# pranoyr/attention-models

Hardware: AMD Instinct MI355X
Metric: ViTVQGAN 256px train-step images/sec (higher is better)
Workload: dtype f32; 1 GPU; BASELINE.json configs[2]: ViTVQGAN dim=256 patch=8 img=256 depth=6+6 h=8 d=64 mlp=2048 (SwiGLU), codebook 8192x32; GAN train step (D phase + G phase, gradient penalty, per_loss_weight=0), Adam, clip 1.0; global_batch=32, batch_per_gpu=32, parallelism=dp1

## Files before the change

attention-models_amd/amk/dense.py:

```python
import ctypes

import torch

from . import lib as _lib
from .lib import EPI_BIAS, EPI_RESID, EPI_SWIGLU, EPI_SWIGLU_BWD, GEMM_NN, GEMM_NT, GEMM_TN, GemmDesc


def _p(t):
    return ctypes.c_void_p(t.data_ptr()) if t is not None else ctypes.c_void_p(0)


def _stream():
    return ctypes.c_void_p(torch.cuda.current_stream().cuda_stream)


def _mat(t, what):
    if t is None:
        return None
    if not t.is_cuda:
        raise RuntimeError("amk ops run only on MI355X (HIP) tensors; got a CPU tensor. There is no CPU fallback.")
    if t.dtype != torch.float32:
        raise RuntimeError(f"amk kernels compute in fp32; got {t.dtype} for {what}")
    if t.dim() != 2:
        raise RuntimeError(f"{what} must be a matrix, got shape {tuple(t.shape)}")
# ... 175 lines not shown
        rows.append([src, R, K, H, blk, dst_w, dst_wt, NR])
        spans.append((dst_w, nw, dst_wt, nt))
        blk += (_pad32(R) // 32) * (_pad32(K) // 32)
    return torch.tensor(rows, dtype=torch.int64).view(-1, 8), blk, off, spans


def x6_split_table(flat, table_dev, n_blocks, planes):
    rc = _lib.load().amk_gemm_x6_split_table(_p(flat), flat.numel(), _p(table_dev), table_dev.shape[0], n_blocks,
                                             _p(planes), planes.numel(), _stream())
    _lib.check(rc, "amk_gemm_x6_split_table")


def gemm_x6_nt(a, planes, N, bias=None, *, a2=None, planes2=None):
    a, a2 = _mat(a, "a"), _mat(a2, "a2")
    M, K = a.shape
    c = torch.empty((M, N), device=a.device, dtype=torch.float32)
    L = _lib.load()
    if a2 is not None:
        if bias is not None or a2.shape[0] != M:
            raise RuntimeError("gemm_x6_nt: the two-segment form takes no bias and equal row counts")
        rc = L.amk_gemm_x6_nt2(_p(a), a.stride(0), _p(planes), K, _p(a2), a2.stride(0), _p(planes2), a2.shape[1],
                               _p(c), N, M, N, _stream())
        _lib.check(rc, "amk_gemm_x6_nt2")
        return c
    rc = L.amk_gemm_x6_nt(_p(a), a.stride(0), _p(planes), _p(_vec(bias, N, "bias")), _p(c), N, M, N, K, _stream())
    _lib.check(rc, "amk_gemm_x6_nt")
    return c


def gemm_x6_nt_swiglu(a, gate_planes, H, b12=None, *, keep_ab=True):
    a = _mat(a, "a")
    M, K = a.shape
    gate = torch.empty((M, H), device=a.device, dtype=torch.float32)
    ab = torch.empty((M, 2 * H), device=a.device, dtype=torch.float32) if keep_ab else None
    rc = _lib.load().amk_gemm_x6_nt_swiglu(_p(a), a.stride(0), _p(gate_planes), _p(_vec(b12, 2 * H, "b12")), _p(gate), H,
                                           _p(ab), 2 * H, M, H, K, _stream())
    _lib.check(rc, "amk_gemm_x6_nt_swiglu")
    return gate, ab


def gemm_x6_nt_swiglu_bwd(dy, w3t_planes, ab):
    dy, ab = _mat(dy, "dy"), _mat(ab, "ab")
    M, K = dy.shape
    H = ab.shape[1] // 2
    if ab.shape != (M, 2 * H):
        raise RuntimeError(f"gemm_x6_nt_swiglu_bwd: (a | b) {tuple(ab.shape)} against dy {tuple(dy.shape)}")
    d_ab = torch.empty((M, 2 * H), device=dy.device, dtype=torch.float32)
    rc = _lib.load().amk_gemm_x6_nt_swiglu_bwd(_p(dy), dy.stride(0), _p(w3t_planes), _p(ab), ab.stride(0), _p(d_ab), 2 * H,
                                               M, H, K, _stream())
    _lib.check(rc, "amk_gemm_x6_nt_swiglu_bwd")
    return d_ab


def _mat16(t, what):
    if not t.is_cuda:
        raise RuntimeError("amk ops run only on MI355X (HIP) tensors; got a CPU tensor. There is no CPU fallback.")
    if t.dtype != torch.bfloat16 or t.dim() != 2:
        raise RuntimeError(f"{what} must be a bf16 matrix, got {t.dtype} {tuple(t.shape)}")
    if t.stride(1) != 1 or t.stride(0) % 8 or t.data_ptr() % 16:
        t = t.contiguous()
    return t


def supported_bf16(N, K):
    return N > 0 and K > 0 and N % 8 == 0 and K % 8 == 0


def gemm_tn_bf16(y, x, want_bias=False, out=None, bias_out=None):
    y, x = _mat16(y, "y"), _mat16(x, "x")
    M, N = y.shape
    K = x.shape[1]
    if x.shape[0] != M:
        raise RuntimeError(f"gemm_tn_bf16: y has {M} rows, x {x.shape[0]}")
    if not supported_bf16(N, K):
        raise RuntimeError(f"gemm_tn_bf16: N and K must be multiples of 8, got {N}, {K}")
    L = _lib.load()
    dw = _out(out, (N, K), "gemm_tn_bf16 out")
    if dw is None:
        dw = torch.empty(N, K, device=y.device, dtype=torch.float32)
    db = None
    if want_bias:
        db = _out(bias_out, (N,), "gemm_tn_bf16 bias_out")
        if db is None:
            db = torch.empty(N, device=y.device, dtype=torch.float32)
    nbytes = L.amk_gemm_tn_bf16_ws_bytes(M, N, K)
    ws = torch.empty(nbytes // 4, device=y.device, dtype=torch.float32) if nbytes else None
    rc = L.amk_gemm_tn_bf16(_p(y), y.stride(0), _p(x), x.stride(0), _p(dw), K, _p(db), M, N, K, _p(ws), nbytes, _stream())
    _lib.check(rc, "amk_gemm_tn_bf16")
    return dw, db


def _bias32(bias, n):
    if bias is None:
        return None
    if bias.dtype != torch.float32 or not bias.is_cuda:
        raise RuntimeError("gemm bf16: the bias stays in fp32 (it is added to the fp32 accumulators)")
    bias = bias.contiguous()
    if bias.numel() != n or bias.data_ptr() % 16:
        raise RuntimeError(f"gemm bf16: bias of {bias.numel()} elements (16-byte aligned) expected {n}")
    return bias


def gemm_nt_bf16(a, w, bias=None):
    a, w = _mat16(a, "a"), _mat16(w, "w")
    (M, K), N = a.shape, w.shape[0]
    if w.shape[1] != K or not supported_bf16(N, K):
# ... 47 lines not shown
```

attention-models_amd/amk/lib.py:

```python
import ctypes
import os
import re

_HERE = os.path.dirname(os.path.abspath(__file__))
LIB_PATH = os.environ.get("AMK_LIB") or os.path.join(_HERE, "libamk.so")
HEADER_PATH = os.path.normpath(os.path.join(_HERE, "..", "..", "include", "amk.h"))

AMK_OK = 0

_c = ctypes
_P = _c.c_void_p
_I = _c.c_int
_L = _c.c_int64
_F = _c.c_float



class GemmDesc(_c.Structure):
    _fields_ = [("op", _c.c_int32), ("epilogue", _c.c_int32), ("m", _L),
                ("n", _c.c_int32), ("k", _c.c_int32), ("split", _c.c_int32), ("reserved", _c.c_int32),
                ("a", _P), ("a2", _P), ("w", _P), ("w2", _P), ("c", _P), ("c2", _P),
                ("lda", _L), ("lda2", _L), ("ldw", _L), ("ldw2", _L), ("ldc", _L), ("ldc2", _L),
                ("bias", _P), ("bias2", _P), ("resid", _P), ("ldr", _L),
                ("ln_mean", _P), ("ln_rstd", _P), ("ln_gamma", _P), ("ln_beta", _P),
# ... 6 lines not shown
SIGNATURES = {
    "amk_version": (_I, []),
    "amk_arch": (_c.c_char_p, []),
    "amk_last_error": (_c.c_char_p, []),
    "amk_attn_fwd": (_I, [_P] * 7 + [_I] * 5 + [_L] * 12 + [_F, _P]),
    "amk_attn_scores_bytes": (_L, [_I, _I, _I, _I]),
    "amk_attn_fwd_keep": (_I, [_P] * 8 + [_I] * 5 + [_L] * 12 + [_F, _P]),
    "amk_attn_fwd_x6_ws_bytes": (_L, [_I, _I, _I]),
    "amk_attn_fwd_x6": (_I, [_P] * 8 + [_I] * 5 + [_L] * 12 + [_F, _P]),
    "amk_attn_fwd_x6_keep": (_I, [_P] * 9 + [_I] * 5 + [_L] * 12 + [_F, _P]),
    "amk_attn_decode_ws_floats": (_L, [_I, _I, _I, _I]),
    "amk_attn_decode": (_I, [_P] * 9 + [_I] * 4 + [_L] * 9 + [_F, _P]),
    "amk_attn_decode_bf16": (_I, [_P] * 9 + [_I] * 4 + [_L] * 9 + [_F, _P]),
    "amk_gemm_rows_bf16": (_I, [_P, _L, _P, _L, _P, _P, _L, _I, _I, _I, _I, _P]),
    "amk_attn_bwd_ws_floats": (_L, [_I, _I, _I, _I, _I]),
    "amk_attn_bwd": (_I, [_P] * 12 + [_I] * 5 + [_L] * 24 + [_F, _I, _P]),
    "amk_attn_bwd_kept": (_I, [_P] * 13 + [_I] * 5 + [_L] * 24 + [_F, _I, _P]),
    "amk_vq_num_partials": (_L, [_L]),
    "amk_vq_lookup_fwd": (_I, [_P, _P, _L, _I, _I, _I] + [_P] * 9 + [_P]),
    "amk_vq_lookup_bwd": (_I, [_P] * 7 + [_F, _L, _I, _I, _P, _P, _P]),
    "amk_vq_lookup_bwd_rows": (_I, [_P] * 7 + [_F, _L, _I, _I, _P, _P, _P]),
    "amk_vq_padded_codes": (_I, [_I, _I]),
    "amk_vq_gather": (_I, [_P, _P, _L, _I, _I, _P, _P, _P]),
    "amk_agent_num_chunks": (_I, [_I]),
    "amk_agent_ws_floats": (_L, [_I, _I, _I, _I, _I]),
    "amk_agent_num_chunks_dh": (_I, [_I, _I]),
    "amk_agent_ws_floats_dh": (_L, [_I, _I, _I, _I, _I, _I]),
    "amk_agent_attn_fwd": (_I, [_P] * 10 + [_I] * 5 + [_L] * 12 + [_F, _P]),
    "amk_agent_attn_bwd": (_I, [_P] * 14 + [_I] * 5 + [_L] * 21 + [_F, _P]),
    "amk_agent_conv_grad_reduce": (_I, [_P, _P, _L, _I, _P, _P, _P]),
    "amk_agent_bf16_ws_floats": (_L, [_I, _I, _I, _I, _I, _I]),
    "amk_agent_attn_bf16_fwd": (_I, [_P] * 10 + [_I] * 5 + [_L] * 12 + [_F, _P]),
    "amk_agent_attn_bf16_bwd": (_I, [_P] * 14 + [_I] * 5 + [_L] * 21 + [_F, _P]),
    "amk_rowsum_num_partials": (_I, [_L]),
    "amk_add_layernorm_fwd": (_I, [_P, _P, _P, _P, _L, _I, _F, _P, _P, _P, _P, _P]),
    "amk_add_layernorm_bwd": (_I, [_P, _P, _P, _P, _P, _P, _L, _I, _P, _P, _P]),
    "amk_colsum": (_I, [_P, _L, _I, _P, _P]),
    "amk_swiglu_fwd": (_I, [_P, _L, _I, _P, _P]),
    "amk_swiglu_bwd": (_I, [_P, _P, _L, _I, _P, _P]),
    "amk_geglu_fwd": (_I, [_P, _L, _I, _P, _P]),
    "amk_geglu_bwd": (_I, [_P, _P, _L, _I, _P, _P]),
    "amk_opt_num_partials": (_I, []),
    "amk_sumsq_partials": (_I, [_P, _L, _P, _P]),
    "amk_adam_flat_step": (_I, [_P] * 4 + [_L, _P, _P, _P, _I] + [_F] * 6 + [_I, _P, _P]),
    "amk_adam_flat_step_shadow": (_I, [_P] * 4 + [_L, _P, _P, _P, _I] + [_F] * 6 + [_I, _P, _P, _P]),
    "amk_gemm_x6_planes_bytes": (_L, [_I, _I]),
    "amk_gemm_x6_split": (_I, [_P, _L, _I, _I, _P, _P]),
    "amk_gemm_x6_nt": (_I, [_P, _L, _P, _P, _P, _L, _I, _I, _I, _P]),
    "amk_gemm_x6_nt2": (_I, [_P, _L, _P, _I, _P, _L, _P, _I, _P, _L, _I, _I, _P]),
    "amk_gemm_x6_gate_rows": (_I, [_I]),
    "amk_gemm_x6_nt_swiglu": (_I, [_P, _L, _P, _P, _P, _L, _P, _L, _I, _I, _I, _P]),
    "amk_gemm_x6_nt_swiglu_bwd": (_I, [_P, _L, _P, _P, _L, _P, _L, _I, _I, _I, _P]),
    "amk_gemm_x6_split_table": (_I, [_P, _L, _P, _I, _L, _P, _L, _P]),
    "amk_gemm_f32_ws_bytes": (_L, [_c.POINTER(GemmDesc)]),
    "amk_gemm_f32": (_I, [_c.POINTER(GemmDesc), _P, _L, _P]),
    "amk_row_stats": (_I, [_P, _L, _I, _F, _P, _P, _P]),
    "amk_attn_bf16_fwd": (_I, [_P] * 7 + [_I] * 5 + [_L] * 12 + [_F, _P]),
    "amk_attn_bf16_bwd_ws_floats": (_L, [_I, _I, _I, _I]),
    "amk_attn_bf16_bwd": (_I, [_P] * 12 + [_I] * 5 + [_L] * 24 + [_F, _P]),
    "amk_swiglu_bf16_fwd": (_I, [_P, _L, _I, _P, _P]),
    "amk_swiglu_bf16_bwd": (_I, [_P, _P, _L, _I, _P, _P]),
    "amk_add_layernorm_mixed_fwd": (_I, [_P, _I, _P, _P, _P, _L, _I, _F, _P, _P, _P, _P, _P]),
    "amk_add_layernorm_mixed_bwd": (_I, [_P, _I, _P, _P, _P, _P, _P, _L, _I, _P, _P, _P, _P]),
    "amk_geglu_ln_bf16_num_partials": (_I, [_L, _I]),
    "amk_geglu_ln_bf16_fwd": (_I, [_P, _L, _L, _I, _P, _P, _F, _P, _P, _P, _P]),
    "amk_geglu_ln_bf16_bwd": (_I, [_P, _L, _P, _P, _P, _P, _L, _I, _P, _P, _P]),
    "amk_gemm_bf16": (_I, [_I, _I, _P, _L, _P, _L, _P, _P, _L, _P, _L, _L, _I, _I, _P]),
    "amk_gemm_bf16_swiglu_bwd": (_I, [_P, _L, _P, _L, _P, _L, _P, _L, _L, _I, _I, _P]),
    "amk_gemm_tn_bf16_ws_bytes": (_L, [_L, _I, _I]),
    "amk_gemm_tn_bf16": (_I, [_P, _L, _P, _L, _P, _L, _P, _L, _I, _I, _P, _L, _P]),
    "amk_sample_step": (_I, [_P, _P, _F, _P, _c.c_uint64, _c.c_uint64, _F, _L, _I, _I, _P, _F, _P, _P, _P]),
    "amk_moe_route_ws_ints": (_L, [_L, _I, _I]),
    "amk_moe_route": (_I, [_P, _L, _I, _I] + [_P] * 8),
    "amk_grouped_gemm_nt": (_I, [_P, _L, _I, _P, _P, _P, _P, _L, _I, _I, _I, _P, _P]),
    "amk_grouped_gemm_nn": (_I, [_P, _L, _I, _P, _P, _P, _P, _L, _I, _I, _I, _P, _P]),
    "amk_grouped_gemm_nt_acc": (_I, [_P, _L, _I, _P, _P, _P, _P, _L, _I, _I, _I, _P, _I, _P]),
    "amk_grouped_gemm_nn_acc": (_I, [_P, _L, _I, _P, _P, _P, _P, _L, _I, _I, _I, _P, _I, _P]),
    "amk_grouped_gemm_wgrad": (_I, [_P, _L, _I, _P, _L, _I, _P, _P, _P, _L, _I, _I, _I, _P, _P, _P]),
    "amk_moe_combine": (_I, [_P, _P, _P, _L, _I, _I, _I, _P, _P]),
    "amk_moe_expert_sums": (_I, [_P, _L, _I, _P, _P, _L, _I, _I, _I, _P, _P]),
    "amk_moe_topk": (_I, [_P, _L, _I, _I, _P, _P, _P]),
    "amk_moe_route_distinct": (_I, [_P, _L, _I, _I, _P, _P, _P, _P]),
    "amk_moe_combine_rows": (_I, [_P, _P, _P, _L, _I, _I, _I, _I, _I, _P, _P]),
    "amk_moe_gate_grad_rows": (_I, [_P, _P, _P, _P, _L, _I, _I, _I, _I, _I, _P, _P]),
    "amk_moe_gate_grad": (_I, [_P, _P, _P, _P, _L, _I, _I, _I, _I, _P, _P]),
    "amk_bnact_ws_floats": (_L, [_I, _I, _L]),
    "amk_bnact_fwd": (_I, [_P, _P, _P, _I, _I, _L, _F, _F, _F] + [_P] * 7),
    "amk_bnact_bwd": (_I, [_P] * 6 + [_I, _I, _L, _F] + [_P] * 6),
    "amk_bnact_bwd_bwd": (_I, [_P] * 10 + [_I, _I, _L, _F] + [_P] * 5),
    "amk_bnact_bf16_fwd": (_I, [_P, _P, _P, _I, _I, _L, _F, _F, _F] + [_P] * 7),
    "amk_bnact_bf16_bwd": (_I, [_P] * 6 + [_I, _I, _L, _F] + [_P] * 6),
    "amk_bnact_bf16_bwd_bwd": (_I, [_P] * 10 + [_I, _I, _L, _F] + [_P] * 5),
    "amk_gnact_ws_floats": (_L, [_I, _I, _L, _I]),
    "amk_gnact_fwd": (_I, [_P, _P, _P, _I, _I, _L, _I, _F, _I] + [_P] * 5),
    "amk_gnact_bwd": (_I, [_P] * 6 + [_I, _I, _L, _I, _I] + [_P] * 5),
    "amk_gnact_bf16_ws_floats": (_L, [_I, _I, _L, _I]),
    "amk_gnact_bf16_fwd": (_I, [_P, _P, _P, _I, _I, _L, _I, _F, _I] + [_P] * 5),
    "amk_gnact_bf16_bwd": (_I, [_P] * 6 + [_I, _I, _L, _I, _I] + [_P] * 5),
    "amk_ce_head_fwd_ws_bytes": (_L, [_L, _I, _I]),
    "amk_ce_head_bwd_ws_bytes": (_L, [_L, _I, _I]),
    "amk_ce_head_fwd": (_I, [_P, _L, _P, _L, _P, _L, _L, _I, _I, _P, _P, _P, _P, _P, _L, _P]),
    "amk_ce_head_bwd": (_I, [_P, _L, _P, _L, _P, _L, _L, _I, _I, _P, _P, _P, _P, _P, _L, _P, _L, _P, _L, _P]),
    "amk_ce_head_bias_fwd": (_I, [_P, _L, _P, _L, _P, _P, _L, _L, _I, _I, _P, _P, _P, _P, _P, _L, _P]),
    "amk_ce_head_bias_bwd": (_I, [_P, _L, _P, _L, _P, _P, _L, _L, _I, _I, _P, _P, _P, _P, _P, _L, _P, _L, _P, _P, _L, _P]),
    "amk_ce_head_bf16_fwd_ws_bytes": (_L, [_L, _I, _I]),
    "amk_ce_head_bf16_bwd_ws_bytes": (_L, [_L, _I, _I]),
# ... 48 lines not shown
```

attention-models_amd/amk/ops.py:

```python
import ctypes
import os
import weakref

import torch
from torch.autograd.function import once_differentiable

from . import lib as _lib

_NULL = ctypes.c_void_p(0)


def _ptr(t):
    return ctypes.c_void_p(t.data_ptr()) if t is not None else _NULL


def _stream():
    return ctypes.c_void_p(torch.cuda.current_stream().cuda_stream)


KERNEL_EVENTS = None


class _timed:

# ... 1507 lines not shown
    if not _ln_supported(x.shape[-1]) or x.numel() == 0 or not x.is_cuda:
        return torch.nn.functional.layer_norm(x, (x.shape[-1],), weight, bias, eps)
    if branch and _mixed_ln():
        with torch.autocast("cuda", enabled=False):
            return _AddLayerNormMixed.apply(x, None, weight, bias, eps)[1]
    return _LayerNorm.apply(x, weight, bias, eps)


def add_layer_norm(x, res, weight, bias, eps=1e-5, branch=False):
    if not _ln_supported(x.shape[-1]) or x.numel() == 0 or not x.is_cuda:
        h = x + res
        return h, torch.nn.functional.layer_norm(h, (h.shape[-1],), weight, bias, eps)
    if branch and _mixed_ln():
        with torch.autocast("cuda", enabled=False):
            return _AddLayerNormMixed.apply(x, res.float(), weight, bias, eps)
    return _AddLayerNorm.apply(x, res, weight, bias, eps)


def colsum(x2):
    M, N = x2.shape
    if N % 4 != 0 or N > 1024:
        return x2.sum(0)
    x2 = _c16(x2)
    L = _lib.load()
    part = torch.empty((L.amk_rowsum_num_partials(M), N), device=x2.device, dtype=torch.float32)
    _lib.check(L.amk_colsum(_ptr(x2), M, N, _ptr(part), _stream()), "amk_colsum")
    return part.sum(0)


class _BiasLinear(torch.autograd.Function):

    @staticmethod
    def forward(ctx, x, weight, bias):
        _require_device(x, weight, bias)
        ctx.save_for_backward(x, weight)
        return torch.nn.functional.linear(x, weight, bias)

    @staticmethod
    @once_differentiable
    def backward(ctx, dy):
        x, weight = ctx.saved_tensors
        dy2 = dy.contiguous().view(-1, dy.shape[-1])
        dx = dy2.mm(weight).view(x.shape) if ctx.needs_input_grad[0] else None
        dw = dy2.t().mm(x.reshape(-1, x.shape[-1])) if ctx.needs_input_grad[1] else None
        db = colsum(dy2) if ctx.needs_input_grad[2] else None
        return dx, dw, db


GEMM_MODE = os.environ.get("AMK_GEMM", "auto")
if GEMM_MODE not in ("auto", "f32", "bf16x6"):
    raise RuntimeError(f"AMK_GEMM must be auto, f32 or bf16x6 (got {GEMM_MODE!r})")
X6_LINEAR = os.environ.get("AMK_X6_LINEAR", "1") != "0"
X6_AUTO_KINDS = frozenset(k for k in os.environ.get("AMK_X6_KINDS", "linear,linear2,ffn").split(",") if k)
X6_AUTO_FORMS = frozenset(k for k in os.environ.get("AMK_X6_FORMS", "fwd").split(",") if k)


def gemm_x6_nt(a2, b2, bias=None):
    _require_device(a2, b2, bias)
    if a2.stride(1) != 1:
        a2 = a2.contiguous()
    if b2.stride(1) != 1:
        b2 = b2.contiguous()
    M, K = a2.shape
    N = b2.shape[0]
    L = _lib.load()
    planes = torch.empty((L.amk_gemm_x6_planes_bytes(N, K),), device=a2.device, dtype=torch.uint8)
    c = torch.empty((M, N), device=a2.device, dtype=torch.float32)
    with _timed(f"gemm_x6_nt M{M} N{N} K{K}"):
        _lib.check(L.amk_gemm_x6_split(_ptr(b2), b2.stride(0), N, K, _ptr(planes), _stream()), "amk_gemm_x6_split")
        rc = L.amk_gemm_x6_nt(_ptr(a2), a2.stride(0), _ptr(planes), _ptr(bias), _ptr(c), N, M, N, K, _stream())
    _lib.check(rc, "amk_gemm_x6_nt")
    return c


def _x6_ok(x, weight):
    K = weight.shape[1]
    if K % 4 or x.numel() == 0 or x.data_ptr() % 16 or weight.data_ptr() % 16:
        return False
    if x.stride(-1) != 1 or (x.dim() >= 2 and x.stride(-2) % 4):
        return False
    return x.numel() * 4 < 0x7ffffff0 and weight.numel() * 8 < 0x7ffffff0


class _LinearX6(torch.autograd.Function):

    @staticmethod
    def forward(ctx, x, weight, bias):
        _require_device(x, weight, bias)
        x2 = x.reshape(-1, x.shape[-1])
        ctx.save_for_backward(x2, weight)
        ctx.x_shape = x.shape
        ctx.has_bias = bias is not None
        return gemm_x6_nt(x2, weight, bias).view(*x.shape[:-1], weight.shape[0])

    @staticmethod
    @once_differentiable
    def backward(ctx, dy):
        x2, weight = ctx.saved_tensors
        dy2 = dy.contiguous().view(-1, dy.shape[-1])
        dx = dw = db = None
        if ctx.needs_input_grad[0]:
            N = weight.shape[0]
            if N % 4 == 0:
                dx = gemm_x6_nt(dy2, weight.t().contiguous()).view(ctx.x_shape)
            else:
                dx = dy2.mm(weight).view(ctx.x_shape)
        if ctx.needs_input_grad[1]:
            dw = dy2.t().mm(x2)
        if ctx.has_bias and ctx.needs_input_grad[2]:
            db = colsum(dy2)
        return dx, dw, db


def _x6_planes(kind, x, *weights, gate=None):
    if GEMM_MODE != "auto" or not X6_LINEAR or kind not in X6_AUTO_KINDS or torch.is_autocast_enabled():
        return None
    if not x.is_cuda or x.dtype != torch.float32 or x.numel() == 0 or x.shape[-1] % 4:
        return None
    if kind == "linear" and min(weights[0].shape) < 128:
        return None
    out = []
    for w in weights:
        pl = getattr(w, "_amk_x6", None)
        if pl is None or w._version != w._amk_x6_version or pl.gate != (w is gate) or (pl.R, pl.K) != tuple(w.shape):
            return None
        out.append(pl)
    return tuple(out)


class _X6Linear(torch.autograd.Function):

    @staticmethod
    def forward(ctx, x, weight, bias, pl):
        from . import dense

        x2 = x.reshape(-1, x.shape[-1])
        ctx.save_for_backward(x2, weight)
        ctx.x_shape, ctx.has_bias, ctx.params, ctx.pl = x.shape, bias is not None, (weight, bias), pl
        return dense.gemm_x6_nt(x2, pl.w, pl.R, bias).view(*x.shape[:-1], pl.R)

    @staticmethod
    @once_differentiable
    def backward(ctx, dy):
        from . import dense

        x2, weight = ctx.saved_tensors
        dy2 = dy.reshape(-1, dy.shape[-1])
        dx = dw = db = None
        if ctx.needs_input_grad[0]:
            dx = (dense.gemm_x6_nt(dy2, ctx.pl.wt, ctx.pl.K) if ctx.pl.wt is not None else _nn_plain(dy2, weight)).view(ctx.x_shape)
        if ctx.needs_input_grad[1] or (ctx.has_bias and ctx.needs_input_grad[2]):
            want_b = ctx.has_bias and ctx.needs_input_grad[2]
            dw, db = _tn_into(dense.gemm_tn, dy2, x2, ctx.params[0], ctx.params[1] if want_b else None)
        return dx, dw, db, None


class _X6Linear2(torch.autograd.Function):

    @staticmethod
    def forward(ctx, x, wa, wb, pa, pb):
        from . import dense

        x2 = x.reshape(-1, x.shape[-1])
        ctx.save_for_backward(x2, wa, wb)
        ctx.x_shape, ctx.params, ctx.pl = x.shape, (wa, wb), (pa, pb)
        a, b = dense.gemm_x6_nt(x2, pa.w, pa.R), dense.gemm_x6_nt(x2, pb.w, pb.R)
        return a.view(*x.shape[:-1], pa.R), b.view(*x.shape[:-1], pb.R)

    @staticmethod
    @once_differentiable
    def backward(ctx, da, db_):
        from . import dense

        x2, wa, wb = ctx.saved_tensors
        pa, pb = ctx.pl
        da2 = da.reshape(-1, da.shape[-1])
        db2 = db_.reshape(-1, db_.shape[-1])
        dx = None
        if ctx.needs_input_grad[0]:
            dx = (dense.gemm_x6_nt(da2, pa.wt, pa.K, a2=db2, planes2=pb.wt) if pa.wt is not None and pb.wt is not None
                  else dense.gemm_nn(da2, wa, a2=db2, w2=wb)).view(ctx.x_shape)
        dwa = dwb = None
        if ctx.needs_input_grad[1] or ctx.needs_input_grad[2]:
            (ar, av), (br, bv) = _claim(ctx.params[0]), _claim(ctx.params[1])
            dwa, dwb, _ = dense.gemm_tn(da2, x2, y2=db2, out=av, out2=bv)
            if av is not None:
                ar.wrote(ctx.params[0])
                dwa = None
            if bv is not None:
                br.wrote(ctx.params[1])
                dwb = None
        return dx, dwa, dwb, None, None


class _X6SwiGLUFFN(torch.autograd.Function):

    @staticmethod
    def forward(ctx, x, w12, b12, w3, b3, p12, p3):
        from . import dense

        x2 = x.reshape(-1, x.shape[-1])
        need = any(ctx.needs_input_grad)
        gate, ab = dense.gemm_x6_nt_swiglu(x2, p12.w, p12.R // 2, b12, keep_ab=need)
        out = dense.gemm_x6_nt(gate, p3.w, p3.R, b3)
        if need:
            ctx.save_for_backward(x2, w12, w3, ab, gate)
        ctx.x_shape, ctx.has_bias, ctx.params, ctx.pl = x.shape, (b12 is not None, b3 is not None), (w12, b12, w3, b3), (p12, p3)
        return out.view(*x.shape[:-1], p3.R)

    @staticmethod
    @once_differentiable
    def backward(ctx, dout):
        from . import dense

        x2, w12, w3, ab, gate = ctx.saved_tensors
        p12, p3 = ctx.pl
        d2 = dout.reshape(-1, dout.shape[-1])
        d_ab = dense.gemm_x6_nt_swiglu_bwd(d2, p3.wt, ab) if p3.wt is not None else dense.gemm_nn(d2, w3, swiglu_ab=ab)
        dw3, db3 = _tn_into(dense.gemm_tn, d2, gate, ctx.params[2], ctx.params[3] if ctx.has_bias[1] else None)
        dx = None
        if ctx.needs_input_grad[0]:
            dx = (dense.gemm_x6_nt(d_ab, p12.wt, p12.K) if p12.wt is not None else _nn_plain(d_ab, w12)).view(ctx.x_shape)
        dw12, db12 = _tn_into(dense.gemm_tn, d_ab, x2, ctx.params[0], ctx.params[1] if ctx.has_bias[0] else None)
        return dx, dw12, db12, dw3, db3, None, None


DENSE_MODE = os.environ.get("AMK_DENSE", "auto")


DENSE_AUTO_MAX_K = int(os.environ.get("AMK_DENSE_MAX_K", "512"))


def _dense_ok(x, *weights):
    if DENSE_MODE == "lib" or torch.is_autocast_enabled() or not x.is_cuda or x.dtype != torch.float32 or x.numel() == 0:
        return False
    if x.shape[-1] % 4 or x.shape[-1] < 128:
        return False
    if DENSE_MODE == "auto" and x.shape[-1] > DENSE_AUTO_MAX_K:
        return False
    return all(w.dtype == torch.float32 and w.shape[0] % 4 == 0 and w.shape[0] >= 128 and w.is_contiguous() for w in weights)


def _nn_plain(dy2, weight):
    from . import dense

    if DENSE_MODE == "amk":
        return dense.gemm_nn(dy2, weight)
    return dy2.mm(weight)


def _claim(p):
    ref = getattr(p, "_amk_reducer", None) if p is not None else None
    red = ref() if ref is not None else None
    if red is None:
        return None, None
    view = red.claim(p)
    return (red, view) if view is not None else (None, None)


class _DenseLinear(torch.autograd.Function):

    @staticmethod
    def forward(ctx, x, weight, bias):
        from . import dense

        x2 = x.reshape(-1, x.shape[-1])
        ctx.save_for_backward(x2, weight)
        ctx.x_shape = x.shape
        ctx.has_bias = bias is not None
        ctx.params = (weight, bias)
        if DENSE_MODE == "auto" and weight.shape[0] < 512:
            return torch.nn.functional.linear(x, weight, bias)
        return dense.gemm_nt(x2, weight, bias).view(*x.shape[:-1], weight.shape[0])

    @staticmethod
    @once_differentiable
# ... 748 lines not shown
```

include/amk.h:

```cpp
#ifndef AMK_H_
#define AMK_H_

#include <stdint.h>

#ifdef __cplusplus
extern "C" {
#endif

#define AMK_VERSION 140

enum {
  AMK_OK = 0,
  AMK_EINVAL = -1,
  AMK_EUNSUPPORTED = -2,
  AMK_ELAUNCH = -3
};

int amk_version(void);
const char* amk_arch(void);
const char* amk_last_error(void);

int amk_attn_fwd(const float* q, const float* k, const float* v, float* o, float* stats,
                 const uint8_t* key_mask, const uint8_t* causal_mask,
                 int B, int H, int I, int J, int D,
// ... 188 lines not shown
                            const float* agents, const float* vagent, const float* stats1,
                            void* dq, void* dk, void* dv, float* ws, float* dconvw_part, float* dconvb_part,
                            int B, int H, int T, int D, int P,
                            int64_t q_sb, int64_t q_st, int64_t q_sh, int64_t k_sb, int64_t k_st, int64_t k_sh,
                            int64_t v_sb, int64_t v_st, int64_t v_sh, int64_t do_sb, int64_t do_st, int64_t do_sh,
                            int64_t dq_sb, int64_t dq_st, int64_t dq_sh, int64_t dk_sb, int64_t dk_st, int64_t dk_sh,
                            int64_t dv_sb, int64_t dv_st, int64_t dv_sh, float scale, void* stream);

int amk_rowsum_num_partials(int64_t M);
int amk_add_layernorm_fwd(const float* x, const float* res, const float* gamma, const float* beta,
                          int64_t M, int D, float eps, float* h, float* y, float* mean, float* rstd, void* stream);
int amk_add_layernorm_bwd(const float* dy, const float* h, const float* dh_in, const float* gamma,
                          const float* mean, const float* rstd, int64_t M, int D, float* dh, float* dgb_part,
                          void* stream);
int amk_colsum(const float* x, int64_t M, int N, float* part, void* stream);

int amk_swiglu_fwd(const float* ab, int64_t M, int H, float* out, void* stream);
int amk_swiglu_bwd(const float* ab, const float* d_out, int64_t M, int H, float* d_ab, void* stream);

int amk_geglu_fwd(const float* ab, int64_t M, int H, float* out, void* stream);
int amk_geglu_bwd(const float* ab, const float* d_out, int64_t M, int H, float* d_ab, void* stream);

int amk_opt_num_partials(void);
int amk_sumsq_partials(const float* x, int64_t n, float* partials, void* stream);
int amk_adam_flat_step(float* param, float* grad, float* exp_avg, float* exp_avg_sq, int64_t n,
                       const int32_t* seg_param, const float* param_tab,
                       const float* partials, int n_partials,
                       float max_norm, float lr, float beta1, float beta2, float eps, float weight_decay,
                       int decoupled, float* norm_out, void* stream);
int amk_adam_flat_step_shadow(float* param, float* grad, float* exp_avg, float* exp_avg_sq, int64_t n,
                              const int32_t* seg_param, const float* param_tab,
                              const float* partials, int n_partials,
                              float max_norm, float lr, float beta1, float beta2, float eps, float weight_decay,
                              int decoupled, float* norm_out, void* param_bf16, void* stream);

int amk_sample_step(const float* logits, const float* null_logits, float cfg_scale,
                    const float* gumbel, uint64_t seed, uint64_t offset, float tau,
                    int64_t R, int V, int keep, const uint8_t* mask, float unmasked_score,
                    int64_t* ids, float* scores, void* stream);

int64_t amk_gemm_x6_planes_bytes(int N, int K);
int amk_gemm_x6_split(const float* W, int64_t ldw, int N, int K, void* planes, void* stream);
int amk_gemm_x6_nt(const float* A, int64_t lda, const void* w_planes, const float* bias,
                   float* C, int64_t ldc, int M, int N, int K, void* stream);
int amk_gemm_x6_nt2(const float* A, int64_t lda, const void* planes, int K, const float* A2, int64_t lda2,
                    const void* planes2, int K2, float* C, int64_t ldc, int M, int N, void* stream);
int amk_gemm_x6_gate_rows(int H);
int amk_gemm_x6_nt_swiglu(const float* A, int64_t lda, const void* gate_planes, const float* bias, float* gate,
                          int64_t ldg, float* ab, int64_t ldab, int M, int H, int K, void* stream);
int amk_gemm_x6_nt_swiglu_bwd(const float* dY, int64_t ldy, const void* w3t_planes, const float* ab, int64_t ldab,
                              float* d_ab, int64_t ldd, int M, int H, int K, void* stream);
int amk_gemm_x6_split_table(const float* flat, int64_t flat_elems, const void* table, int n_entries, int64_t n_blocks,
                            void* planes, int64_t planes_elems, void* stream);

enum { AMK_GEMM_NT = 0, AMK_GEMM_NN = 1, AMK_GEMM_TN = 2 };
enum { AMK_EPI_BIAS = 0, AMK_EPI_RESID = 1, AMK_EPI_SWIGLU = 2, AMK_EPI_SWIGLU_BWD = 3 };
typedef struct amk_gemm_desc {
  int32_t op, epilogue;
  int64_t m;
  int32_t n, k, split, reserved;
  const float *a, *a2, *w, *w2;
  float *c, *c2;
  int64_t lda, lda2, ldw, ldw2, ldc, ldc2;
  const float *bias, *bias2, *resid;
  int64_t ldr;
  const float *ln_mean, *ln_rstd, *ln_gamma, *ln_beta;
  const float* ab;
  int64_t ldab;
  float* gate;
  int64_t ldg;
  float* dbias;
} amk_gemm_desc;
int64_t amk_gemm_f32_ws_bytes(const amk_gemm_desc* d);
int amk_gemm_f32(const amk_gemm_desc* d, void* workspace, int64_t ws_bytes, void* stream);
int amk_row_stats(const float* x, int64_t M, int D, float eps, float* mean, float* rstd, void* stream);

int amk_attn_bf16_fwd(const void* q, const void* k, const void* v, void* o, float* stats,
                      const uint8_t* key_mask, const uint8_t* causal_mask,
                      int B, int H, int I, int J, int D,
                      int64_t q_sb, int64_t q_st, int64_t q_sh, int64_t k_sb, int64_t k_st, int64_t k_sh,
                      int64_t v_sb, int64_t v_st, int64_t v_sh, int64_t o_sb, int64_t o_st, int64_t o_sh,
                      float scale, void* stream);
int64_t amk_attn_bf16_bwd_ws_floats(int B, int H, int I, int J);
int amk_attn_bf16_bwd(const void* q, const void* k, const void* v, const void* o, const float* stats, const void* d_o,
                      void* dq, void* dk, void* dv, float* ws,
                      const uint8_t* key_mask, const uint8_t* causal_mask,
                      int B, int H, int I, int J, int D,
                      int64_t q_sb, int64_t q_st, int64_t q_sh, int64_t k_sb, int64_t k_st, int64_t k_sh,
                      int64_t v_sb, int64_t v_st, int64_t v_sh, int64_t o_sb, int64_t o_st, int64_t o_sh,
                      int64_t do_sb, int64_t do_st, int64_t do_sh, int64_t dq_sb, int64_t dq_st, int64_t dq_sh,
                      int64_t dk_sb, int64_t dk_st, int64_t dk_sh, int64_t dv_sb, int64_t dv_st, int64_t dv_sh,
                      float scale, void* stream);

int amk_swiglu_bf16_fwd(const void* ab, int64_t M, int H, void* out, void* stream);
int amk_swiglu_bf16_bwd(const void* ab, const void* d_out, int64_t M, int H, void* d_ab, void* stream);
int amk_add_layernorm_mixed_fwd(const void* x, int x_is_bf16, const float* res, const float* gamma, const float* beta,
                                int64_t M, int D, float eps, float* h, void* y_bf16, float* mean, float* rstd, void* stream);
int amk_add_layernorm_mixed_bwd(const void* dy, int dy_is_bf16, const float* h, const float* dh_in, const float* gamma,
                                const float* mean, const float* rstd, int64_t M, int D, float* dh, void* dh_bf16,
                                float* dgb_part, void* stream);

int amk_geglu_ln_bf16_num_partials(int64_t M, int H);
int amk_geglu_ln_bf16_fwd(const void* ab, int64_t ab_stride, int64_t M, int H, const float* gamma, const float* beta,
                          float eps, void* y, float* mean, float* rstd, void* stream);
int amk_geglu_ln_bf16_bwd(const void* ab, int64_t ab_stride, const void* dy, const float* gamma, const float* mean,
                          const float* rstd, int64_t M, int H, void* d_ab, float* dgb_part, void* stream);
// ... 111 lines not shown
```

Before: 321.1 images/s.

## Add split-bf16x6 MFMA weight-gradient TN GEMM with M-chunked reduction

```diff
diff --git a/attention-models_amd/amk/dense.py b/attention-models_amd/amk/dense.py
--- a/attention-models_amd/amk/dense.py
+++ b/attention-models_amd/amk/dense.py
@@ -251,6 +251,41 @@
     return d_ab
 
 
+def x6_tn_chunks(M, N, K):
+    nbytes = _lib.load().amk_gemm_x6_tn_ws_bytes(M, N, K)
+    return nbytes // ((N * K + N) * 4) if nbytes else 1
+
+
+def gemm_x6_tn(y, x, *, y2=None, want_bias=False, out=None, out2=None, bias_out=None):
+    y, x, y2 = _mat(y, "y"), _mat(x, "x"), _mat(y2, "y2")
+    M, N1 = y.shape
+    K = x.shape[1]
+    N2 = y2.shape[1] if y2 is not None else 0
+    if x.shape[0] != M or (y2 is not None and y2.shape[0] != M):
+        raise RuntimeError(f"gemm_x6_tn: y {tuple(y.shape)} against x {tuple(x.shape)}")
+    dw = _out(out, (N1, K), "gemm_x6_tn out")
+    if dw is None:
+        dw = torch.empty((N1, K), device=y.device, dtype=torch.float32)
+    dw2 = None
+    if y2 is not None:
+        dw2 = _out(out2, (N2, K), "gemm_x6_tn out2")
+        if dw2 is None:
+            dw2 = torch.empty((N2, K), device=y.device, dtype=torch.float32)
+    db = None
+    if want_bias:
+        db = _out(bias_out, (N1 + N2,), "gemm_x6_tn bias_out")
+        if db is None:
+            db = torch.empty((N1 + N2,), device=y.device, dtype=torch.float32)
+    L = _lib.load()
+    N = N1 + N2
+    nbytes = L.amk_gemm_x6_tn_ws_bytes(M, N, K)
+    ws = torch.empty((nbytes // 4,), device=y.device, dtype=torch.float32) if nbytes else None
+    rc = L.amk_gemm_x6_tn(_p(y), y.stride(0), _p(y2), y2.stride(0) if y2 is not None else 0, N1 if y2 is not None else 0,
+                          _p(x), x.stride(0), _p(dw), K, _p(dw2), K, _p(db), M, N, K, _p(ws), nbytes, _stream())
+    _lib.check(rc, "amk_gemm_x6_tn")
+    return dw, dw2, db
+
+
 def _mat16(t, what):
     if not t.is_cuda:
         raise RuntimeError("amk ops run only on MI355X (HIP) tensors; got a CPU tensor. There is no CPU fallback.")
diff --git a/attention-models_amd/amk/lib.py b/attention-models_amd/amk/lib.py
--- a/attention-models_amd/amk/lib.py
+++ b/attention-models_amd/amk/lib.py
@@ -82,6 +82,8 @@
     "amk_gemm_x6_nt_swiglu": (_I, [_P, _L, _P, _P, _P, _L, _P, _L, _I, _I, _I, _P]),
     "amk_gemm_x6_nt_swiglu_bwd": (_I, [_P, _L, _P, _P, _L, _P, _L, _I, _I, _I, _P]),
     "amk_gemm_x6_split_table": (_I, [_P, _L, _P, _I, _L, _P, _L, _P]),
+    "amk_gemm_x6_tn_ws_bytes": (_L, [_L, _I, _I]),
+    "amk_gemm_x6_tn": (_I, [_P, _L, _P, _L, _I, _P, _L, _P, _L, _P, _L, _P, _L, _I, _I, _P, _L, _P]),
     "amk_gemm_f32_ws_bytes": (_L, [_c.POINTER(GemmDesc)]),
     "amk_gemm_f32": (_I, [_c.POINTER(GemmDesc), _P, _L, _P]),
     "amk_row_stats": (_I, [_P, _L, _I, _F, _P, _P, _P]),
diff --git a/attention-models_amd/amk/ops.py b/attention-models_amd/amk/ops.py
--- a/attention-models_amd/amk/ops.py
+++ b/attention-models_amd/amk/ops.py
@@ -1583,7 +1583,23 @@
     raise RuntimeError(f"AMK_GEMM must be auto, f32 or bf16x6 (got {GEMM_MODE!r})")
 X6_LINEAR = os.environ.get("AMK_X6_LINEAR", "1") != "0"
 X6_AUTO_KINDS = frozenset(k for k in os.environ.get("AMK_X6_KINDS", "linear,linear2,ffn").split(",") if k)
-X6_AUTO_FORMS = frozenset(k for k in os.environ.get("AMK_X6_FORMS", "fwd").split(",") if k)
+X6_AUTO_FORMS = frozenset(k for k in os.environ.get("AMK_X6_FORMS", "fwd,dw").split(",") if k)
+
+
+def _x6_tn_ok(M, N, K, *lds):
+    if M < 1 or N % 4 or K % 4 or any(ld % 4 for ld in lds):
+        return False
+    return all((M + 96) * ld * 4 < (1 << 30) for ld in lds) and N * K * 4 < (1 << 30)
+
+
+def _x6_tn(y, x, **kw):
+    from . import dense
+
+    y2 = kw.get("y2")
+    if "dw" in X6_AUTO_FORMS and _x6_tn_ok(y.shape[0], y.shape[1] + (y2.shape[1] if y2 is not None else 0), x.shape[1],
+                                           *(t.stride(0) for t in (y, x, y2) if t is not None and t.stride(1) == 1)):
+        return dense.gemm_x6_tn(y, x, **kw)
+    return dense.gemm_tn(y, x, **kw)
 
 
 def gemm_x6_nt(a2, b2, bias=None):
@@ -1682,7 +1698,7 @@
             dx = (dense.gemm_x6_nt(dy2, ctx.pl.wt, ctx.pl.K) if ctx.pl.wt is not None else _nn_plain(dy2, weight)).view(ctx.x_shape)
         if ctx.needs_input_grad[1] or (ctx.has_bias and ctx.needs_input_grad[2]):
             want_b = ctx.has_bias and ctx.needs_input_grad[2]
-            dw, db = _tn_into(dense.gemm_tn, dy2, x2, ctx.params[0], ctx.params[1] if want_b else None)
+            dw, db = _tn_into(_x6_tn, dy2, x2, ctx.params[0], ctx.params[1] if want_b else None)
         return dx, dw, db, None
 
 
@@ -1714,7 +1730,7 @@
         dwa = dwb = None
         if ctx.needs_input_grad[1] or ctx.needs_input_grad[2]:
             (ar, av), (br, bv) = _claim(ctx.params[0]), _claim(ctx.params[1])
-            dwa, dwb, _ = dense.gemm_tn(da2, x2, y2=db2, out=av, out2=bv)
+            dwa, dwb, _ = _x6_tn(da2, x2, y2=db2, out=av, out2=bv)
             if av is not None:
                 ar.wrote(ctx.params[0])
                 dwa = None
@@ -1748,11 +1764,11 @@
         p12, p3 = ctx.pl
         d2 = dout.reshape(-1, dout.shape[-1])
         d_ab = dense.gemm_x6_nt_swiglu_bwd(d2, p3.wt, ab) if p3.wt is not None else dense.gemm_nn(d2, w3, swiglu_ab=ab)
-        dw3, db3 = _tn_into(dense.gemm_tn, d2, gate, ctx.params[2], ctx.params[3] if ctx.has_bias[1] else None)
+        dw3, db3 = _tn_into(_x6_tn, d2, gate, ctx.params[2], ctx.params[3] if ctx.has_bias[1] else None)
         dx = None
         if ctx.needs_input_grad[0]:
             dx = (dense.gemm_x6_nt(d_ab, p12.wt, p12.K) if p12.wt is not None else _nn_plain(d_ab, w12)).view(ctx.x_shape)
-        dw12, db12 = _tn_into(dense.gemm_tn, d_ab, x2, ctx.params[0], ctx.params[1] if ctx.has_bias[0] else None)
+        dw12, db12 = _tn_into(_x6_tn, d_ab, x2, ctx.params[0], ctx.params[1] if ctx.has_bias[0] else None)
         return dx, dw12, db12, dw3, db3, None, None
 
 
diff --git a/attention-models_amd/csrc/gemm_x6_tn.hip b/attention-models_amd/csrc/gemm_x6_tn.hip
--- /dev/null
+++ b/attention-models_amd/csrc/gemm_x6_tn.hip
@@ -0,0 +1,330 @@
+#include "amk_common.h"
+#include <stdlib.h>
+
+namespace amk_x6tn {
+
+typedef __bf16 bf16x8 __attribute__((ext_vector_type(8)));
+typedef __bf16 bf16x4 __attribute__((ext_vector_type(4)));
+typedef short s16x4 __attribute__((ext_vector_type(4)));
+
+constexpr unsigned COL_PAST = 0x40000000u;
+
+struct Params {
+  const float *y, *y2, *x;
+  float *c, *c2, *dbias, *ws, *dbias_ws;
+  int64_t M, ldy, ldy2, ldx, ldc, ldc2;
+  int N, K, split, ntk, total, nchunk, steps_per_chunk;
+};
+
+__device__ __forceinline__ void lds_barrier() {
+  __builtin_amdgcn_fence(__ATOMIC_RELEASE, "workgroup", "local");
+  __builtin_amdgcn_s_barrier();
+  __builtin_amdgcn_fence(__ATOMIC_ACQUIRE, "workgroup", "local");
+}
+
+__device__ __forceinline__ f32x16 zero16() {
+  f32x16 z;
+#pragma unroll
+  for (int i = 0; i < 16; ++i) z[i] = 0.f;
+  return z;
+}
+
+__device__ __forceinline__ void split4(const float4& x, bf16x4 (&pl)[3]) {
+  const float v[4] = {x.x, x.y, x.z, x.w};
+#pragma unroll
+  for (int j = 0; j < 4; ++j) {
+    const __bf16 h = (__bf16)v[j];
+    const float r1 = v[j] - (float)h;
+    const __bf16 m = (__bf16)r1;
+    pl[0][j] = h; pl[1][j] = m; pl[2][j] = (__bf16)(r1 - (float)m);
+  }
+}
+
+__device__ __forceinline__ bf16x4 tr_read(const __bf16* p) {
+  const s16x4 v = __builtin_amdgcn_ds_read_tr16_b64_v4i16((__attribute__((address_space(3))) s16x4*)p);
+  return __builtin_bit_cast(bf16x4, v);
+}
+template <int STRIDE>
+__device__ __forceinline__ bf16x8 tr_frag(const __bf16* img, int r0, int c0, int lane) {
+  const int hf = lane >> 5, grp = (lane >> 4) & 1, q = (lane & 15) >> 2, pp = lane & 3;
+  const __bf16* a = img + (r0 + 8 * hf + q) * STRIDE + c0 + 16 * grp + 4 * pp;
+  const bf16x4 lo = tr_read(a), hi = tr_read(a + 4 * STRIDE);
+  bf16x8 r;
+#pragma unroll
+  for (int i = 0; i < 4; ++i) { r[i] = lo[i]; r[4 + i] = hi[i]; }
+  return r;
+}
+
+template <int NWN, int NWK, int BKM>
+__global__ __launch_bounds__(64 * NWN * NWK) void gemm_x6_tn_kernel(Params p) {
+  constexpr int NTH = 64 * NWN * NWK, TN = 64 * NWN, TK = 64 * NWK;
+  constexpr int YSTR = TN + 32, XSTR = TK + 32;
+  constexpr int YPL = BKM * YSTR, XPL = BKM * XSTR;
+  constexpr int XT = 3 * YPL, STAGE = 3 * YPL + 3 * XPL;
+  constexpr int YCG = TN / 4, YRP = NTH / YCG, YNP = BKM / YRP;
+  constexpr int XCG = TK / 4, XRP = NTH / XCG, XNP = BKM / XRP;
+  static_assert(TN == 128 && TK % 128 == 0 && BKM % 16 == 0 && YNP >= 1 && XNP >= 1 && YNP * YRP == BKM && XNP * XRP == BKM, "tile shape");
+  static_assert(YRP * TN * 4 <= STAGE * 2, "the bias fold fits the first stage");
+  extern __shared__ __attribute__((aligned(16))) __bf16 smem[];
+  const int tid = threadIdx.x, lane = tid & 63, wave = __builtin_amdgcn_readfirstlane(tid >> 6), ln = lane & 31, hf = lane >> 5;
+  const int wn = wave / NWK, wk = wave % NWK;
+  const int u = xcd_remap(blockIdx.x, p.total);
+  const int tk = u % p.ntk, rest = u / p.ntk;
+  const int tn = rest / p.nchunk, chunk = rest - tn * p.nchunk;
+  int n0 = tn * TN;
+  const int k0 = tk * TK;
+  const bool seg = p.split > 0 && n0 >= p.split;
+  const float* Yb = seg ? p.y2 : p.y;
+  const int64_t ldy = seg ? p.ldy2 : p.ldy;
+  const int nrows = p.split > 0 ? (seg ? p.N - p.split : p.split) : p.N;
+  if (seg) n0 -= p.split;
+  const int64_t mbeg = (int64_t)chunk * p.steps_per_chunk * BKM;
+  int64_t mend = mbeg + (int64_t)p.steps_per_chunk * BKM;
+  if (mend > p.M) mend = p.M;
+  const int mrows = (int)(mend - mbeg);
+  const int nk = ((mrows + BKM - 1) / BKM + 1) & ~1;
+
+  const int ycg = tid % YCG, ysr = tid / YCG, xcg = tid % XCG, xsr = tid / XCG;
+  const __amdgpu_buffer_rsrc_t y_rsrc = __builtin_amdgcn_make_buffer_rsrc((void*)(Yb + mbeg * ldy), 0, (int)(((int64_t)(mrows - 1) * ldy + nrows) * 4), 0x00020000);
+  const __amdgpu_buffer_rsrc_t x_rsrc = __builtin_amdgcn_make_buffer_rsrc((void*)(p.x + mbeg * p.ldx), 0, (int)(((int64_t)(mrows - 1) * p.ldx + p.K) * 4), 0x00020000);
+  const bool yok = n0 + 4 * ycg < nrows, xok = k0 + 4 * xcg < p.K;
+  unsigned yoff[YNP], xoff[XNP];
+#pragma unroll
+  for (int i = 0; i < YNP; ++i) yoff[i] = yok ? (unsigned)(((int64_t)(ysr + YRP * i) * ldy + n0 + 4 * ycg) * 4) : COL_PAST;
+#pragma unroll
+  for (int i = 0; i < XNP; ++i) xoff[i] = xok ? (unsigned)(((int64_t)(xsr + XRP * i) * p.ldx + k0 + 4 * xcg) * 4) : COL_PAST;
+  const unsigned ystep = (unsigned)(BKM * ldy * 4), xstep = (unsigned)(BKM * p.ldx * 4);
+  struct Stg { float4 y[YNP], x[XNP]; };
+  auto gload = [&](Stg& g, int t) {
+#pragma unroll
+    for (int i = 0; i < YNP; ++i)
+      g.y[i] = __builtin_bit_cast(float4, __builtin_amdgcn_raw_buffer_load_b128(y_rsrc, (int)(yoff[i] == COL_PAST ? COL_PAST : yoff[i] + (unsigned)t * ystep), 0, 0));
+#pragma unroll
+    for (int i = 0; i < XNP; ++i)
+      g.x[i] = __builtin_bit_cast(float4, __builtin_amdgcn_raw_buffer_load_b128(x_rsrc, (int)(xoff[i] == COL_PAST ? COL_PAST : xoff[i] + (unsigned)t * xstep), 0, 0));
+  };
+  const bool do_bias = p.dbias != nullptr && tk == 0;
+  float4 bsum = make_float4(0.f, 0.f, 0.f, 0.f);
+  auto lstore = [&](__bf16* stage, const Stg& g) {
+#pragma unroll
+    for (int i = 0; i < YNP; ++i) {
+      const float4 v = g.y[i];
+      if (do_bias) { bsum.x += v.x; bsum.y += v.y; bsum.z += v.z; bsum.w += v.w; }
+      bf16x4 pl[3];
+      split4(v, pl);
+#pragma unroll
+      for (int q = 0; q < 3; ++q) *reinterpret_cast<bf16x4*>(&stage[q * YPL + (ysr + YRP * i) * YSTR + 4 * ycg]) = pl[q];
+    }
+#pragma unroll
+    for (int i = 0; i < XNP; ++i) {
+      bf16x4 pl[3];
+      split4(g.x[i], pl);
+#pragma unroll
+      for (int q = 0; q < 3; ++q) *reinterpret_cast<bf16x4*>(&stage[XT + q * XPL + (xsr + XRP * i) * XSTR + 4 * xcg]) = pl[q];
+    }
+  };
+  f32x16 acc[2][2];
+#pragma unroll
+  for (int i = 0; i < 2; ++i)
+#pragma unroll
+    for (int j = 0; j < 2; ++j) acc[i][j] = zero16();
+  Stg ga, gb;
+  gload(ga, 0);
+  gload(gb, 1);
+  lstore(smem, ga);
+  gload(ga, 2);
+  lds_barrier();
+  auto step = [&](int t, Stg& g) {
+    const __bf16* cur = smem + (t & 1) * STAGE;
+    lstore(smem + ((t + 1) & 1) * STAGE, g);
+    gload(g, t + 3);
+#pragma unroll
+    for (int s = 0; s < BKM / 16; ++s) {
+      bf16x8 a[2][3], b[2][3];
+#pragma unroll
+      for (int q = 0; q < 3; ++q) {
+#pragma unroll
+        for (int i = 0; i < 2; ++i) {
+          a[i][q] = tr_frag<YSTR>(cur + q * YPL, 16 * s, 64 * wn + 32 * i, lane);
+          b[i][q] = tr_frag<XSTR>(cur + XT + q * XPL, 16 * s, 64 * wk + 32 * i, lane);
+        }
+      }
+      constexpr int PA[6] = {1, 2, 0, 1, 0, 0};
+      constexpr int PB[6] = {1, 0, 2, 0, 1, 0};
+#pragma unroll
+      for (int q = 0; q < 6; ++q)
+#pragma unroll
+        for (int i = 0; i < 2; ++i)
+#pragma unroll
+          for (int j = 0; j < 2; ++j) acc[i][j] = __builtin_amdgcn_mfma_f32_32x32x16_bf16(a[i][PA[q]], b[j][PB[q]], acc[i][j], 0, 0, 0);
+    }
+    lds_barrier();
+  };
+  for (int t = 0; t < nk; t += 2) {
+    step(t, gb);
+    step(t + 1, ga);
+  }
+  float* Cb;
+  int64_t ldc;
+  if (p.nchunk > 1) { Cb = p.ws + ((int64_t)chunk * p.N + (seg ? p.split : 0)) * p.K; ldc = p.K; }
+  else { Cb = seg ? p.c2 : p.c; ldc = seg ? p.ldc2 : p.ldc; }
+#pragma unroll
+  for (int i = 0; i < 2; ++i) {
+#pragma unroll
+    for (int j = 0; j < 2; ++j) {
+      const int kc = k0 + 64 * wk + 32 * j + ln;
+      if (kc < p.K) {
+#pragma unroll
+        for (int r = 0; r < 16; ++r) {
+          const int n = n0 + 64 * wn + 32 * i + acc_row(r, hf);
+          if (n < nrows) Cb[(int64_t)n * ldc + kc] = acc[i][j][r];
+        }
+      }
+    }
+  }
+  if (do_bias) {
+    float* red = reinterpret_cast<float*>(smem);
+    *reinterpret_cast<float4*>(&red[ysr * TN + 4 * ycg]) = bsum;
+    lds_barrier();
+    if (tid < TN) {
+      float s = 0.f;
+#pragma unroll
+      for (int r = 0; r < YRP; ++r) s += red[r * TN + tid];
+      const int n = n0 + tid;
+      if (n < nrows) (p.nchunk > 1 ? p.dbias_ws + (int64_t)chunk * p.N : p.dbias)[(seg ? p.split : 0) + n] = s;
+    }
+  }
+}
+
+__global__ __launch_bounds__(256) void x6_tn_reduce_kernel(Params p) {
+  const int64_t total4 = (int64_t)p.N * p.K / 4, slab = (int64_t)p.N * p.K;
+  const int64_t i = (int64_t)blockIdx.x * 256 + threadIdx.x;
+  if (i < total4) {
+    const float* src = p.ws + 4 * i;
+    float4 s = make_float4(0.f, 0.f, 0.f, 0.f);
+    int c = 0;
+    for (; c + 8 <= p.nchunk; c += 8) {
+      float4 v[8];
+#pragma unroll
+      for (int j = 0; j < 8; ++j) v[j] = *reinterpret_cast<const float4*>(src + (c + j) * slab);
+#pragma unroll
+      for (int j = 0; j < 8; ++j) { s.x += v[j].x; s.y += v[j].y; s.z += v[j].z; s.w += v[j].w; }
+    }
+    for (; c < p.nchunk; ++c) {
+      const float4 v = *reinterpret_cast<const float4*>(src + c * slab);
+      s.x += v.x; s.y += v.y; s.z += v.z; s.w += v.w;
+    }
+    const int64_t e = 4 * i, row = e / p.K;
+    const int col = (int)(e - row * p.K);
+    if (p.split > 0 && row >= p.split) *reinterpret_cast<float4*>(p.c2 + (row - p.split) * p.ldc2 + col) = s;
+    else *reinterpret_cast<float4*>(p.c + row * p.ldc + col) = s;
+  }
+  if (p.dbias && blockIdx.x == gridDim.x - 1) {
+    for (int n = threadIdx.x; n < p.N; n += 256) {
+      float s = 0.f;
+      for (int c = 0; c < p.nchunk; ++c) s += p.dbias_ws[(int64_t)c * p.N + n];
+      p.dbias[n] = s;
+    }
+  }
+}
+
+}
+
+using namespace amk_x6tn;
+
+static int x6tn_tile_k(int N, int K) {
+  static int forced = -1;
+  if (forced < 0) {
+    const char* e = getenv("AMK_X6_TN_TK");
+    forced = e ? atoi(e) : 0;
+  }
+  if (forced == 128 || forced == 256) return forced;
+  return (K >= 256 && ((N + 127) / 128) * ((K + 255) / 256) >= 12) ? 256 : 128;
+}
+
+static int x6tn_step_rows(int TK) { return TK == 256 ? 16 : 32; }
+
+static int x6tn_chunks(int64_t M, int N, int K, int* spc) {
+  static int cus = 0;
+  if (cus == 0) {
+    int dev = 0;
+    if (hipGetDevice(&dev) != hipSuccess || hipDeviceGetAttribute(&cus, hipDeviceAttributeMultiprocessorCount, dev) != hipSuccess || cus <= 0) cus = 256;
+  }
+  const int TK = x6tn_tile_k(N, K), BKM = x6tn_step_rows(TK);
+  const int tiles = ((N + 127) / 128) * ((K + TK - 1) / TK);
+  const int64_t steps = (M + BKM - 1) / BKM, min_steps = 256 / BKM;
+  int64_t chunks = cus / tiles;
+  if (chunks < 1) chunks = 1;
+  if (chunks > steps / min_steps) chunks = steps / min_steps > 0 ? steps / min_steps : 1;
+  const int64_t s = (steps + chunks - 1) / chunks;
+  chunks = (steps + s - 1) / s;
+  *spc = (int)s;
+  return (int)chunks;
+}
+
+extern "C" int64_t amk_gemm_x6_tn_ws_bytes(int64_t M, int N, int K) {
+  if (M <= 0 || N <= 0 || K <= 0) return 0;
+  int spc;
+  const int chunks = x6tn_chunks(M, N, K, &spc);
+  return chunks > 1 ? ((int64_t)chunks * N * K + (int64_t)chunks * N) * 4 : 0;
+}
+
+extern "C" int amk_gemm_x6_tn(const float* y, int64_t ldy, const float* y2, int64_t ldy2, int split, const float* x, int64_t ldx,
+                              float* c, int64_t ldc, float* c2, int64_t ldc2, float* dbias, int64_t M, int N, int K,
+                              void* workspace, int64_t ws_bytes, void* stream) {
+  AMK_CHECK_ARG(y && x && c, "amk_gemm_x6_tn: null operand");
+  AMK_CHECK_ARG(M > 0 && N > 0 && K > 0, "amk_gemm_x6_tn: non-positive size");
+  const bool two = split > 0;
+  if (two) {
+    AMK_CHECK_ARG(y2 && c2 && split < N, "amk_gemm_x6_tn: second row segment incomplete");
+    AMK_CHECK_SUPPORTED(split % 128 == 0 && ldy2 % 4 == 0 && ldc2 % 4 == 0 && (((uintptr_t)y2 | (uintptr_t)c2) & 15) == 0,
+                        "amk_gemm_x6_tn: split must be a multiple of 128, ldy2 and ldc2 of 4, y2 and c2 16-byte aligned");
+  }
+  AMK_CHECK_SUPPORTED(N % 4 == 0 && K % 4 == 0 && ldy % 4 == 0 && ldx % 4 == 0 && ldc % 4 == 0,
+                      "amk_gemm_x6_tn: N, K and the leading dimensions must be multiples of 4");
+  AMK_CHECK_SUPPORTED((((uintptr_t)y | (uintptr_t)x | (uintptr_t)c) & 15) == 0, "amk_gemm_x6_tn: pointers must be 16-byte aligned");
+  const int64_t lim2 = 0x7ffffff0ll, lim1 = 1ll << 30;
+  AMK_CHECK_SUPPORTED(((M - 1) * ldy + (two ? split : N)) * 4 < lim2 && ((M - 1) * ldx + K) * 4 < lim2 &&
+                      (!two || ((M - 1) * ldy2 + (N - split)) * 4 < lim2) && (int64_t)N * K * 4 < lim1,
+                      "amk_gemm_x6_tn: an operand must span < 2 GiB, the output < 1 GiB");
+  Params p = {};
+  p.y = y; p.y2 = y2; p.x = x; p.c = c; p.c2 = c2; p.dbias = dbias;
+  p.M = M; p.N = N; p.K = K; p.split = two ? split : 0;
+  p.ldy = ldy; p.ldy2 = ldy2; p.ldx = ldx; p.ldc = ldc; p.ldc2 = ldc2;
+  int spc;
+  p.nchunk = x6tn_chunks(M, N, K, &spc);
+  p.steps_per_chunk = spc;
+  const int TK = x6tn_tile_k(N, K), BKM = x6tn_step_rows(TK);
+  AMK_CHECK_SUPPORTED((int64_t)(spc + 3) * BKM * ldy * 4 < lim1 && (int64_t)(spc + 3) * BKM * ldx * 4 < lim1 &&
+                      (!two || (int64_t)(spc + 3) * BKM * ldy2 * 4 < lim1), "amk_gemm_x6_tn: chunk panel beyond 1 GiB");
+  if (p.nchunk > 1) {
+    AMK_CHECK_ARG(workspace && ws_bytes >= amk_gemm_x6_tn_ws_bytes(M, N, K) && ((uintptr_t)workspace & 15) == 0,
+                  "amk_gemm_x6_tn: workspace of amk_gemm_x6_tn_ws_bytes() bytes (16-byte aligned) required");
+    p.ws = static_cast<float*>(workspace);
+    p.dbias_ws = p.ws + (int64_t)p.nchunk * N * K;
+  }
+  p.ntk = (K + TK - 1) / TK;
+  const int64_t total = (int64_t)((N + 127) / 128) * p.ntk * p.nchunk;
+  AMK_CHECK_SUPPORTED(total < (1ll << 31), "amk_gemm_x6_tn: grid too large");
+  p.total = (int)total;
+  hipStream_t st = static_cast<hipStream_t>(stream);
+  constexpr size_t lds4 = (size_t)2 * 3 * 32 * ((128 + 32) + (128 + 32)) * 2, lds8 = (size_t)2 * 3 * 16 * ((128 + 32) + (256 + 32)) * 2;
+  static bool attr_set[64] = {};
+  int dev_id = 0;
+  AMK_CHECK_ARG(hipGetDevice(&dev_id) == hipSuccess && dev_id >= 0 && dev_id < 64, "amk_gemm_x6_tn: no current device");
+  if (!attr_set[dev_id]) {
+    AMK_CHECK_SUPPORTED(hipFuncSetAttribute(reinterpret_cast<const void*>(gemm_x6_tn_kernel<2, 2, 32>), hipFuncAttributeMaxDynamicSharedMemorySize, (int)lds4) == hipSuccess &&
+                        hipFuncSetAttribute(reinterpret_cast<const void*>(gemm_x6_tn_kernel<2, 4, 16>), hipFuncAttributeMaxDynamicSharedMemorySize, (int)lds8) == hipSuccess,
+                        "amk_gemm_x6_tn: the device refused %zu bytes of dynamic LDS", lds4);
+    attr_set[dev_id] = true;
+  }
+  if (TK == 256) hipLaunchKernelGGL((gemm_x6_tn_kernel<2, 4, 16>), dim3((unsigned)total), dim3(512), lds8, st, p);
+  else hipLaunchKernelGGL((gemm_x6_tn_kernel<2, 2, 32>), dim3((unsigned)total), dim3(256), lds4, st, p);
+  AMK_CHECK_LAUNCH("amk_gemm_x6_tn");
+  if (p.nchunk > 1) {
+    const int64_t blocks = ((int64_t)N * K / 4 + 255) / 256;
+    hipLaunchKernelGGL(x6_tn_reduce_kernel, dim3((unsigned)blocks), dim3(256), 0, st, p);
+    AMK_CHECK_LAUNCH("amk_gemm_x6_tn(reduce)");
+  }
+  return AMK_OK;
+}
diff --git a/include/amk.h b/include/amk.h
--- a/include/amk.h
+++ b/include/amk.h
@@ -264,6 +264,10 @@
                               float* d_ab, int64_t ldd, int M, int H, int K, void* stream);
 int amk_gemm_x6_split_table(const float* flat, int64_t flat_elems, const void* table, int n_entries, int64_t n_blocks,
                             void* planes, int64_t planes_elems, void* stream);
+int64_t amk_gemm_x6_tn_ws_bytes(int64_t M, int N, int K);
+int amk_gemm_x6_tn(const float* y, int64_t ldy, const float* y2, int64_t ldy2, int split, const float* x, int64_t ldx,
+                   float* c, int64_t ldc, float* c2, int64_t ldc2, float* dbias, int64_t M, int N, int K,
+                   void* workspace, int64_t ws_bytes, void* stream);
 
 enum { AMK_GEMM_NT = 0, AMK_GEMM_NN = 1, AMK_GEMM_TN = 2 };
 enum { AMK_EPI_BIAS = 0, AMK_EPI_RESID = 1, AMK_EPI_SWIGLU = 2, AMK_EPI_SWIGLU_BWD = 3 };
```

After: 331.3 images/s, median of 6. 3.2% higher.
